# Sudaraka88/LDWeaver

Hardware: AMD Instinct MI355X
Metric: MI SNP-pairs/sec (higher is better)
Workload: dtype i8

## Files before the change

### ldweaver_amd/csrc/ldw_apx.hip

```cpp
#include <algorithm>
#include <cmath>
#include <cstdlib>
#include <cstring>

#include "ldw_apx.h"
#include "ldw_dev.h"

using namespace ldw;

namespace ldw {

namespace {
constexpr int64_t APX_PROD_CAP = 12000;
struct ProdTable {
    std::vector<int32_t> val;
    std::vector<uint8_t> a, b;
    ProdTable() {
        std::vector<std::pair<int32_t, std::pair<uint8_t, uint8_t>>> all;
        for (int x = 0; x <= 127; ++x)
            for (int y = x; y <= 127; ++y) all.push_back({x * y, {(uint8_t)x, (uint8_t)y}});
        std::sort(all.begin(), all.end());
        for (auto &e : all)
            if (val.empty() || val.back() != e.first) {
                val.push_back(e.first);
// ... 177 lines not shown
    const u64x2v q = {*reinterpret_cast<const uint64_t *>(lut_bytes + (d & 0xFFFFu)), *reinterpret_cast<const uint64_t *>(lut_bytes + (d >> 16))};
    return __builtin_bit_cast(v4i, q);
}
constexpr int APX_LUT_BYTES = 2048;

template <int MT, int NT>
__device__ __forceinline__ void apx_gemm_epilogue(const ApxGemmArgs &P, v16i (&acc)[MT][NT], int ty, int tx, int lane, const int2 *s_tab, uint8_t *s_bt) {
    constexpr int TH = 32 * MT, TWd = 32 * NT;
    const int frow = lane & 31, fh = lane >> 5;
    int bf[NT];
    if (P.fuse) {
#pragma unroll
        for (int j = 0; j < NT; ++j) bf[j] = (int)P.bin_f[tx * TWd + 32 * j + frow];
        for (int r = lane; r < TH; r += 64) s_bt[r] = P.bin_t[ty * TH + r];
        __builtin_amdgcn_wave_barrier();
        __builtin_amdgcn_s_waitcnt(0);
    }
#pragma unroll
    for (int i = 0; i < MT; ++i) {
        bool store = true;
        if (P.fuse) {
            bool ok = true;
#pragma unroll
            for (int j = 0; j < NT; ++j) ok = ok && bf[j] != 255;
            if (P.sr_mask && P.sr_mask[(int64_t)((ty * TH) / 128) * (P.RFpad / 64) + tx] != 0) ok = false;
            int bt[16];
#pragma unroll
            for (int e = 0; e < 16; ++e) {
                bt[e] = (int)s_bt[32 * i + (e & 3) + 8 * (e >> 2) + 4 * fh];
                ok = ok && bt[e] != 255;
            }
            unsigned int fails = 0;
            const bool eligible = __ballot(!ok) == 0ull;
            if (eligible) {
#pragma unroll
                for (int e = 0; e < 16; ++e)
#pragma unroll
                    for (int j = 0; j < NT; ++j) {
                        const int2 th = s_tab[bt[e] * P.tab_nb + bf[j]];
                        const int n = acc[i][j][e];
                        const bool in = n > th.x && n < th.y;
                        ok = ok && in;
                        if (!in) fails |= 1u << (e * NT + j);
                    }
            }
            if (NT == 2 && P.maybe && eligible && __ballot(!ok) != 0ull) {
                const unsigned int mine = (unsigned int)__popc(fails);
                unsigned int incl = mine;
#pragma unroll
                for (int o = 1; o < 64; o <<= 1) {
                    const unsigned int t = __shfl_up(incl, o);
                    if (lane >= o) incl += t;
                }
                const unsigned int tot = (unsigned int)__builtin_amdgcn_readlane((int)incl, 63);
                if (tot <= (unsigned int)APX_MAYBE_MAX) {
                    unsigned int base = 0;
                    if (lane == 0) base = atomicAdd(P.maybe_n, tot);
                    base = (unsigned int)__builtin_amdgcn_readfirstlane((int)base);
                    unsigned int pos = base + incl - mine;
                    unsigned int f = fails;
                    while (f) {
                        const int b = __builtin_ctz(f);
                        f &= f - 1;
                        const int e = b / NT, j = b % NT;
                        if (pos < P.maybe_cap) {
                            ApxMaybe m;
                            m.trow = (uint32_t)(ty * TH + 32 * i + (e & 3) + 8 * (e >> 2) + 4 * fh);
                            m.fcol = (uint32_t)(tx * TWd + 32 * j + frow);
                            int v = 0;
#pragma unroll
                            for (int ee = 0; ee < 16; ++ee)
#pragma unroll
                                for (int jj = 0; jj < NT; ++jj) v = (ee == e && jj == j) ? acc[i][jj][ee] : v;
                            m.n = v;
                            P.maybe[pos] = m;
                        }
                        ++pos;
                    }
                    ok = true;
                }
            }
#ifdef LDW_ABLATE_GEMM_STORE
            const bool clean = __ballot(bf[0] == 255 || bt[0] == 255) == 0ull || __ballot(!ok) == 0ull;
#else
            const bool clean = __ballot(!ok) == 0ull;
#endif
            if (lane == 0) {
#pragma unroll
                for (int h = 0; h < (NT * 32) / 64; ++h) P.clean[(int64_t)((ty * TH + 32 * i) / 32) * (P.RFpad / 64) + (tx * TWd) / 64 + h] = clean ? 1 : 0;
            }
            store = !clean;
        }
        if (store) {
#pragma unroll
            for (int j = 0; j < NT; ++j) {
                const int fcol = tx * TWd + 32 * j + frow;
#pragma unroll
                for (int e = 0; e < 16; ++e) {
                    const int trow = ty * TH + 32 * i + (e & 3) + 8 * (e >> 2) + 4 * fh;
                    P.G[(int64_t)trow * P.RFpad + fcol] = acc[i][j][e];
                }
            }
        }
    }
}

struct TileSummary {
    int bmin, bmax;
    unsigned fand, forr;
};
__device__ __forceinline__ TileSummary apx_fold_rows(const uint8_t *__restrict__ bins, const uint8_t *__restrict__ flags, int n) {
    TileSummary S{255, 0, 0xFFu, 0u};
    for (int i = 0; i < n; i += 16) {
        const uint4 b = *reinterpret_cast<const uint4 *>(bins + i);
        const unsigned w[4] = {b.x, b.y, b.z, b.w};
#pragma unroll
        for (int k = 0; k < 16; ++k) {
            const int v = (int)((w[k >> 2] >> (8 * (k & 3))) & 0xFFu);
            S.bmin = v < S.bmin ? v : S.bmin;
            S.bmax = v > S.bmax ? v : S.bmax;
        }
        if (flags) {
            const uint4 f = *reinterpret_cast<const uint4 *>(flags + i);
            unsigned a = f.x & f.y & f.z & f.w, o = f.x | f.y | f.z | f.w;
            a &= a >> 16; a &= a >> 8;
            o |= o >> 16; o |= o >> 8;
            S.fand &= a & 0xFFu;
            S.forr |= o & 0xFFu;
        }
    }
    return S;
}

__global__ __launch_bounds__(256) void k_apx_live_tiles(ApxGemmArgs P) {
    constexpr int MT = APX_MT, NT = 2, TH = 32 * MT, TWd = 32 * NT;
    __shared__ unsigned int s_wave[4], s_base;
    const int ty = (int)blockIdx.x, ntx = P.RFpad / TWd;
    const int lane = threadIdx.x & 63, wave = threadIdx.x >> 6;
    const TileSummary T = apx_fold_rows(P.bin_t + (int64_t)ty * TH, P.rflag_t ? P.rflag_t + (int64_t)ty * TH : nullptr, TH);
    unsigned int n_pruned = 0;
    for (int tx0 = 0; tx0 < ntx; tx0 += 256) {
        const int tx = tx0 + (int)threadIdx.x;
        const bool valid = tx < ntx && !(P.lower_only && tx * TWd + TWd - 1 < ty * TH);
        bool pruned = false, all_binned = false;
        if (valid && !(P.sr_mask && P.sr_mask[(int64_t)((ty * TH) / 128) * (P.RFpad / 64) + tx] != 0)) {
            const TileSummary F = apx_fold_rows(P.bin_f + (int64_t)tx * TWd, P.rflag_f ? P.rflag_f + (int64_t)tx * TWd : nullptr, TWd);
            all_binned = T.bmax < P.tab_nb && F.bmax < P.tab_nb;
            if (P.rflag_t) {
                const unsigned kt = T.fand & PF_KIND, kf = F.fand & PF_KIND;
                pruned = kt >= 2u && kt == (T.forr & PF_KIND) && kf >= 2u && kf == (F.forr & PF_KIND) &&
                         ((T.fand & (kf == 2u ? PF_DEAD2 : PF_DEAD3)) != 0u || (F.fand & (kt == 2u ? PF_DEAD2 : PF_DEAD3)) != 0u);
            }
            if (!pruned && all_binned && (T.bmax - T.bmin + 1) * (F.bmax - F.bmin + 1) <= 64) {
                bool ok = true;
                for (int bt = T.bmin; bt <= T.bmax; ++bt)
                    for (int bf = F.bmin; bf <= F.bmax; ++bf) {
                        const int2 th = P.tab[bt * P.tab_nb + bf];
                        ok = ok && th.x < 0 && th.y == 2147483647;
                    }
                pruned = ok;
            }
        }
        if (pruned && all_binned) {
#pragma unroll
            for (int i = 0; i < MT; ++i)
#pragma unroll
                for (int h = 0; h < (NT * 32) / 64; ++h) P.clean[(int64_t)((ty * TH + 32 * i) / 32) * (P.RFpad / 64) + (tx * TWd) / 64 + h] = 1;
        }
        const bool live = valid && !pruned;
        const unsigned long long lm = __ballot(live);
        n_pruned += (unsigned int)__popcll(__ballot(valid && pruned));
        if (lane == 0) s_wave[wave] = (unsigned int)__popcll(lm);
        __syncthreads();
        if (threadIdx.x == 0) {
            const unsigned int tot = s_wave[0] + s_wave[1] + s_wave[2] + s_wave[3];
            s_base = tot ? atomicAdd(P.n_live, tot) : 0u;
        }
        __syncthreads();
        unsigned int off = s_base;
        for (int w = 0; w < wave; ++w) off += s_wave[w];
        if (live) P.tile_list[off + (unsigned int)__popcll(lm & ((1ull << lane) - 1ull))] = (uint32_t)(ty * ntx + tx);
        __syncthreads();
    }
    if (lane == 0 && n_pruned) atomicAdd(P.skip_ctr, (unsigned long long)n_pruned);
}

template <int MT, int NT, bool FINE, int WPS = 2>
__global__ __launch_bounds__(256, WPS) void gemm_apx_kernel(ApxGemmArgs P) {
    extern __shared__ __attribute__((aligned(16))) uint8_t smem[];
    uint64_t *lutFF = reinterpret_cast<uint64_t *>(smem);
    uint8_t *sA = smem + APX_LUT_BYTES, *sB = sA + (size_t)P.M2 * 128;
    int2 *s_tab = reinterpret_cast<int2 *>(sB + (size_t)P.M2 * 128);
    const int tid = threadIdx.x;
    const int lane = tid & 63, wave = __builtin_amdgcn_readfirstlane(tid >> 6);
    constexpr int TH = 32 * MT, TWd = 32 * NT;
    const int ntx = P.RFpad / TWd;
    unsigned int k = 0, k_end = 0, step = 1;
    int t;
    if (P.tile_list) {
        const unsigned int n_live = *P.n_live, nw = gridDim.x * 4u, w = blockIdx.x * 4u + (unsigned int)wave;
        if (blockIdx.x * 4u >= n_live) return;
#ifdef LDW_APX_RUNS_CONTIG
        const unsigned int base = n_live / nw, rem = n_live % nw;
        k = w * base + (w < rem ? w : rem);
        k_end = k + base + (w < rem ? 1u : 0u);
#else
        k = w;
        k_end = n_live;
        step = nw;
#endif
        t = k < k_end ? (int)P.tile_list[k] : -1;
    } else {
        auto outside = [&](int ty, int tx) { return ty * TH >= P.RTpad || tx * TWd >= P.RFpad || (P.lower_only && tx * TWd + TWd - 1 < ty * TH); };
        const int ty0 = 2 * (int)blockIdx.y, tx0 = 2 * (int)blockIdx.x;
        if (outside(ty0, tx0) && outside(ty0, tx0 + 1) && outside(ty0 + 1, tx0) && outside(ty0 + 1, tx0 + 1)) return;
        const int ty = ty0 + (wave >> 1), tx = tx0 + (wave & 1);
        t = outside(ty, tx) ? -1 : ty * ntx + tx;
    }
    if (P.fuse)
        for (int i = tid; i < P.tab_nb * P.tab_nb; i += 256) s_tab[i] = P.tab[i];
    {
        uint64_t e = 0;
#pragma unroll
        for (int k8 = 0; k8 < 8; ++k8) e |= ((tid >> k8) & 1) ? (0xFFull << (8 * k8)) : 0ull;
        lutFF[tid] = e;
        const int n16 = P.M2 * 8;
        for (int i = tid; i < n16; i += 256) {
            reinterpret_cast<uint4 *>(sA)[i] = reinterpret_cast<const uint4 *>(P.dig_a)[i];
            reinterpret_cast<uint4 *>(sB)[i] = reinterpret_cast<const uint4 *>(P.dig_b)[i];
        }
    }
    __syncthreads();
    if (t < 0) return;
    const int frow = lane & 31, fh = lane >> 5;
    const int64_t sta = (int64_t)P.RTpad * 2, stb = (int64_t)P.RFpad * 2;
    const uint8_t *base_t, *base_f;
    const unsigned int lane_off = (unsigned int)(frow * 2 + fh) * 16u;
    auto piece = [&](const uint8_t *base, int64_t macro_step_bytes, int i) {
        return *reinterpret_cast<const apx_u32x4 *>(base + macro_step_bytes + 1024 * i);
    };
    apx_u32x4 wa[MT], wb[NT], na[MT], nb[NT];
    auto open_tile = [&](int ty, int tx) {
        base_t = reinterpret_cast<const uint8_t *>(P.panel_t) + (int64_t)ty * TH * 32 + lane_off;
        base_f = reinterpret_cast<const uint8_t *>(P.panel_f) + (int64_t)tx * TWd * 32 + lane_off;
#pragma unroll
        for (int i = 0; i < MT; ++i) na[i] = piece(base_t, 0, i);
#pragma unroll
        for (int i = 0; i < NT; ++i) nb[i] = piece(base_f, 0, i);
    };
    const uint8_t *lut_bytes = smem;
    int ty = t / ntx, tx = t - ty * ntx;
    open_tile(ty, tx);
    for (;;) {
        k += step;
        const int t_next = k < k_end ? (int)P.tile_list[k] : -1;
        v16i acc[MT][NT];
#pragma unroll
        for (int i = 0; i < MT; ++i)
#pragma unroll
            for (int j = 0; j < NT; ++j)
#pragma unroll
                for (int e = 0; e < 16; ++e) acc[i][j][e] = 0;
        for (int m = 0; m < P.M2; ++m) {
#pragma unroll
            for (int i = 0; i < MT; ++i) wa[i] = na[i];
#pragma unroll
            for (int i = 0; i < NT; ++i) wb[i] = nb[i];
            if (m + 1 < P.M2) {
#pragma unroll
                for (int i = 0; i < MT; ++i) na[i] = piece(base_t, (int64_t)(m + 1) * sta * 16, i);
#pragma unroll
                for (int i = 0; i < NT; ++i) nb[i] = piece(base_f, (int64_t)(m + 1) * stb * 16, i);
            }
            typedef const __attribute__((address_space(4))) v4i *shift_ptr;
            const v4i sh4 = ((shift_ptr)(uintptr_t)P.shift)[m];
            const int shk[4] = {sh4[0], sh4[1], sh4[2], sh4[3]};
            const uint8_t *dA = sA + m * 128 + fh * (FINE ? 16 : 64), *dB = sB + m * 128 + fh * (FINE ? 16 : 64);
            auto kstep = [&](auto KKc) {
                constexpr int kk = decltype(KKc)::value;
                const int sh = shk[kk];
                if ((FINE || kk == 0) && sh) {
#pragma unroll
                    for (int i = 0; i < MT; ++i)
#pragma unroll
                        for (int j = 0; j < NT; ++j)
#pragma unroll
                            for (int e = 0; e < 16; ++e) acc[i][j][e] = (int)((unsigned)acc[i][j][e] >> sh);
                }
                const v4i da = *reinterpret_cast<const v4i *>(dA + (FINE ? 32 : 16) * kk);
                const v4i db = *reinterpret_cast<const v4i *>(dB + (FINE ? 32 : 16) * kk);
                v4i fa[MT], fb[NT];
#pragma unroll
                for (int i = 0; i < MT; ++i) fa[i] = expand16s<kk>(lut_bytes, wa[i]) & da;
#pragma unroll
                for (int i = 0; i < NT; ++i) fb[i] = expand16s<kk>(lut_bytes, wb[i]) & db;
#pragma unroll
                for (int i = 0; i < MT; ++i)
#pragma unroll
                    for (int j = 0; j < NT; ++j) acc[i][j] = __builtin_amdgcn_mfma_i32_32x32x32_i8(fa[i], fb[j], acc[i][j], 0, 0, 0);
            };
            kstep(std::integral_constant<int, 0>{});
            kstep(std::integral_constant<int, 1>{});
            kstep(std::integral_constant<int, 2>{});
            kstep(std::integral_constant<int, 3>{});
        }
        const int ty_next = t_next / ntx, tx_next = t_next - ty_next * ntx;
        if (t_next >= 0) open_tile(ty_next, tx_next);
        int bt_off = wave * 256;
// ... 738 lines not shown
```

### ldweaver_amd/csrc/ldw_mi.hip

```cpp
#include <algorithm>
#include <chrono>
#include <cmath>
#include <cstring>
#include "ldw_prim.h"

#include "ldw_internal.h"
#include "ldw_dev.h"
#ifndef LDW_SCREEN_V
#define LDW_SCREEN_V 2
#endif
#ifndef LDW_SCREEN_WAVES
#define LDW_SCREEN_WAVES 6
#endif
#include "ldw_epi.h"
#include "ldw_pass_plan.h"
#include <future>

#include "ldw_apx.h"

using namespace ldw;

namespace ldw {
#include "ldw_mi_screen.inc"
#include "ldw_mi_eval.inc"
#include "ldw_mi_select.inc"
}

namespace {
#include "ldw_mi_block.inc"
#include "ldw_mi_items.inc"
#include "ldw_mi_pass.inc"
}

namespace ldw {
int ensure_streams(ldw_ctx *c) {
    if (c->streams_ready) return LDW_OK;
    const unsigned quiet = hipEventDisableTiming;
    LDW_HIP(c->copy_stream.ensure(hipStreamNonBlocking));
    for (int k = 0; k < LDW_NSLOT; ++k) {
        LDW_HIP(c->ev_up[k].ensure(quiet));
        LDW_HIP(c->ev_done[k].ensure(quiet));
        LDW_HIP(c->ev_pick[k].ensure(quiet));
        LDW_HIP(c->ev_gemm[k].ensure(quiet));
        if (int rc = c->pin_pick[k].reserve((size_t)LDW_SPAN_MAX * PICK_STRIDE + 64, "ensure_streams")) return rc;
    }
    LDW_HIP(c->ev_lrc.ensure(quiet));
    for (auto &e : c->ev_probe) LDW_HIP(e.ensure(quiet));
    if (int rc = c->pin_lrc.reserve(64, "ensure_streams")) return rc;
    {
        int lo_p = 0, hi_p = 0;
        LDW_HIP(hipDeviceGetStreamPriorityRange(&lo_p, &hi_p));
        LDW_HIP(c->gemm_stream.ensure(hipStreamNonBlocking, lo_p));
    }
    LDW_HIP(c->lr_st.ensure(hipStreamNonBlocking));
    for (auto &e : c->lr_ev) LDW_HIP(e.ensure(quiet));
    if (int rc = c->lr_counts.reserve(sizeof(int64_t) * 64, "ensure_streams")) return rc;
    if (int rc = c->lr_pin.reserve((size_t)32 << 20, "ensure_streams")) return rc;
    c->streams_ready = true;
    return LDW_OK;
}

int join_prepare(ldw_ctx *c) {
    if (!c) return LDW_OK;
    int rc = LDW_OK;
    for (int which = 0; which < 2; ++which) {
        std::thread &t = which == 0 ? c->prep_thread : c->prep_thread2;
        if (t.joinable()) t.join();
        int &trc = which == 0 ? c->prep_rc : c->prep_rc2;
        if (trc != LDW_OK && rc == LDW_OK) {
            rc = trc;
            set_error("side thread of %s: %s", which == 0 ? "ldw_ctx_create" : "ldw_ctx_reserve", (which == 0 ? c->prep_err : c->prep_err2).c_str());
        }
        trc = LDW_OK;
    }
    return rc;
}

int reserve_slot_buffers(ldw_ctx *c, int64_t Npad, int64_t blk, int64_t nseg) {
    const int64_t KW = Npad / 64;
    const SlotGeom g = slot_geom_estimate(blk, nseg);
    const size_t RF = (size_t)g.RFpad, RT = (size_t)g.RTpad;
    const size_t cap = pair_cap_for(g.nf, g.nt, g.nseg);
    const size_t one = (size_t)blk * (size_t)blk;
    for (int s = 0; s < LDW_NSLOT; ++s) {
        if (int rc = c->panel[s][0].reserve(RF * (size_t)KW * 16)) return rc;
        if (int rc = c->panel[s][1].reserve(RT * (size_t)KW * 16)) return rc;
        if (int rc = c->Gapx[s].reserve(RF * RT * 4)) return rc;
        if (int rc = UnitsLayout(g).reserve(c->apx_units[s])) return rc;
        if (int rc = PacksLayout(g).reserve(c->apx_packs[s])) return rc;
        if (int rc = MiniLayout(g).reserve(c->apx_mini[s])) return rc;
        if (int rc = PairsLayout((uint32_t)cap, maybe_cap_for(g.RTpad, g.RFpad)).reserve(c->pairs[s])) return rc;
        if (int rc = BinsLayout(g).reserve(c->apx_bins[s])) return rc;
        if (int rc = c->apx_clean[s].reserve((RT / 32) * (RF / 64) + 64)) return rc;
        if (int rc = c->hist[s].reserve((size_t)nseg * NBINS * 8)) return rc;
        const size_t cand = std::max<size_t>(one, (size_t)nseg * std::min<size_t>(one, (size_t)PAIR_PATHS * PAIR_SHARDS * cap));
        if (int rc = c->cand_key[s].reserve(cand * 8)) return rc;
        if (int rc = c->cand_val[s].reserve(cand * 8)) return rc;
        if (int rc = gx(c, s).reserve(RF * RF * 8)) return rc;
    }
    if (int rc = c->pair_sums.reserve((size_t)PAIR_PATHS * PAIR_SHARDS * cap * 16 * 8)) return rc;
    return LDW_OK;
}

void warm_mi() {
    hipFuncAttributes a;
    (void)hipFuncGetAttributes(&a, reinterpret_cast<const void *>(&k_zero4));
    (void)hipFuncGetAttributes(&a, reinterpret_cast<const void *>(&k_mi_screen<1, true>));
    (void)hipGetLastError();
}
}

extern "C" {

int ldw_mi_block(ldw_ctx *c, const int32_t *from_idx, int64_t nf, const int32_t *to_idx, int64_t nt, int quirk_mode,
                 double *MI_out, int on_device) {
    if (int rc = check_gpu(c)) return rc;
    LDW_REQUIRE(from_idx && to_idx && MI_out, LDW_ERR_ARG, "ldw_mi_block: null argument");
    LDW_REQUIRE(quirk_mode == LDW_QUIRK_REFERENCE || quirk_mode == LDW_QUIRK_INTENDED, LDW_ERR_ARG, "bad quirk mode");
    EmitArgs E;
    memset(&E, 0, sizeof(E));
    if (int rc = run_block_mi(c, from_idx, nf, to_idx, nt, quirk_mode, E)) return rc;
    LDW_HIP(hipMemcpyAsync(MI_out, c->MIblk.p, (size_t)nf * nt * 8, on_device ? hipMemcpyDeviceToDevice : hipMemcpyDeviceToHost,
                           c->stream));
    LDW_HIP(hipStreamSynchronize(c->stream));
    float t01 = 0, t12 = 0;
    LDW_HIP(hipEventElapsedTime(&t01, c->ev[0], c->ev[1]));
    LDW_HIP(hipEventElapsedTime(&t12, c->ev[1], c->ev[2]));
    c->last_ms[0] = t01;
    c->last_ms[1] = t12;
    c->last_ms[2] = 0;
    c->last_ms[3] = t01 + t12;
    return LDW_OK;
}

int ldw_joint_tables(ldw_ctx *c, const int32_t *pair_a, const int32_t *pair_b, int64_t np, int64_t *counts_out,
                     int64_t *fixed_out, int *frac_bits_out) {
    if (int rc = check_gpu(c)) return rc;
    LDW_REQUIRE(pair_a && pair_b && np > 0, LDW_ERR_ARG, "ldw_joint_tables: bad argument");
    if (int rc = join_prepare(c)) return rc;
    if (int rc = ensure_rows(c)) return rc;
    if (frac_bits_out) *frac_bits_out = c->wts.frac_bits;
    const int64_t CH = 1024;
    std::vector<int8_t> ones((size_t)c->Npad, 1);
    ldw::DevBuf d_ones, d_out, d_cmarg;
    int rc = LDW_OK;
    if ((rc = d_ones.reserve((size_t)c->Npad)) || (rc = d_out.reserve((size_t)CH * 25 * 8)) || (rc = d_cmarg.reserve((size_t)c->L * 40))) return rc;
    hipError_t he = hipMemcpyAsync(d_ones.p, ones.data(), ones.size(), hipMemcpyHostToDevice, c->stream);
    if (he != hipSuccess) return ldw::hip_fail(he, "memcpy ones", __FILE__, __LINE__);
    hipLaunchKernelGGL(k_slot_counts, dim3((unsigned)((c->L + 255) / 256)), dim3(256), 0, c->stream,
                       c->rows.counts.as<int32_t>(), c->rows.slot_meta.as<uint32_t>(), c->L, d_cmarg.as<int64_t>());
    for (int64_t p0 = 0; p0 < np && rc == LDW_OK; p0 += CH) {
        const int64_t n = std::min(CH, np - p0);
        SideLists SF, ST;
        if ((rc = build_side(c, pair_a + p0, n, SF))) break;
        if ((rc = build_side(c, pair_b + p0, n, ST))) break;
        const int RFpad = SF.Rpad, RTpad = ST.Rpad;
        if ((rc = upload_i32(c, c->rowlist_f, SF.rowlist)) || (rc = upload_i32(c, c->rowlist_t, ST.rowlist)) ||
            (rc = upload_i32(c, c->lrow_f, SF.lrow)) || (rc = upload_i32(c, c->lrow_t, ST.lrow)))
            break;
        std::vector<int32_t> vf(pair_a + p0, pair_a + p0 + n), vt(pair_b + p0, pair_b + p0 + n);
        if ((rc = upload_i32(c, c->idx_f, vf)) || (rc = upload_i32(c, c->idx_t, vt))) break;
        if (hipStreamSynchronize(c->stream) != hipSuccess) { rc = LDW_ERR_HIP; break; }
        if ((rc = c->G.reserve((size_t)RFpad * RTpad * 8))) break;
        for (int pass = 0; pass < 2 && rc == LDW_OK; ++pass) {
            int64_t *host_out = pass == 0 ? counts_out : fixed_out;
            if (!host_out) continue;
            rc = launch_gemm_bits(c, c->rows.Mbits.as<uint64_t>(), c->KW, c->rowlist_t.as<int32_t>(), RTpad, c->rowlist_f.as<int32_t>(), RFpad, c->G.as<int64_t>(),
                                  pass == 0 ? 1 : c->wts.nlimbs, pass == 0 ? d_ones.as<int8_t>() : c->wts.digits.as<int8_t>(), 0);
// ... 416 lines not shown
```

### ldweaver_amd/csrc/ldw_mi_items.inc

```

struct StageImage {
    struct Part {
        size_t off, bytes;
        const void *src;
        void (*point)(DevPtrs &, const char *);
    };
    Part part[18] = {};
    int n = 0;
    size_t bytes = 0;
    template <class T> static T elem_of(const T *DevPtrs::*);
    template <auto F> using Elem = decltype(elem_of(F));
    template <auto F> size_t array(const Elem<F> *src, size_t count) {
        part[n] = Part{bytes, count * sizeof(Elem<F>), src, [](DevPtrs &D, const char *p) { D.*F = reinterpret_cast<const Elem<F> *>(p); }};
        bytes = (bytes + part[n].bytes + 63) / 64 * 64;
        return part[n++].off;
    }
    void copy_to(char *image) const {
        for (int k = 0; k < n; ++k)
            if (part[k].src && part[k].bytes) memcpy(image + part[k].off, part[k].src, part[k].bytes);
    }
    void bind(DevPtrs &D, const char *image) const {
        for (int k = 0; k < n; ++k) part[k].point(D, image + part[k].off);
    }
};

struct HostBlock {
    int64_t nf = 0, nt = 0, n_sr_blk = 0, n_lr_total = 0, blk_no = 0;
    int RFpad = 0, RTpad = 0, slot = 0;
    bool diag = false, submitted = false;
    bool uploaded = false;
    bool mixed = false;
    bool apx = false;
    bool generic = false;
    int guess = -1;
    LoHost lo;
    StageImage img;
    size_t total = 0;
    DevPtrs D{};
    EmitArgs E{};
    int spec_B = -1;
    int span = 0;
    int32_t seg_start[LDW_SPAN_MAX] = {}, seg_nt[LDW_SPAN_MAX] = {};
    int64_t seg_lr_total[LDW_SPAN_MAX] = {};
    size_t cand_cap = 0;
    SpanSeg sseg[LDW_SPAN_MAX] = {};
    int pin_slot = -1;
    bool force_plain = false;
    bool span_alone = false;
    size_t stage_base = 0;
    int64_t sr_base = 0;
    std::vector<int32_t> span_from, span_to;
};

struct SpanPlan {
    int nseg = 0;
    int32_t start[LDW_SPAN_MAX] = {}, nt[LDW_SPAN_MAX] = {};
};

static inline bool speculation_pays(const ldw_ctx *c, const ldw_mi_params *p) {
    if (c->knobs.path_mode != 0) return true;
    return !(p->lr_links_approx > 0.0) || p->lr_retain_links < 0.007 * p->lr_links_approx;
}

struct PrepWork {
    ldw_ctx *c;
    const int32_t *from_idx, *to_idx;
    int64_t nf, nt;
    HostBlock &hb;
    std::vector<ColInfo> cols;
    std::string cols_err;
    std::future<int> cols_job;
    const std::vector<int32_t> *ord_f = nullptr, *ord_t = nullptr;
    std::vector<int32_t> ord_f_own, ord_t_own, ord_f_full, ord_t_full;
    SideLists SF, ST;
    std::vector<int32_t> pf, cmax, tf;
    std::vector<int64_t> tbase;
    std::vector<uint8_t> band;
    std::vector<uint32_t> bandl;
    int intervals(const ldw_mi_params *p, const SpanPlan *sp);
    int row_order(const SpanPlan *sp);
    void tiles(int slot);
    void band_mask();
    bool band_list();
    int join_cols() {
        const int rc = cols_job.valid() ? cols_job.get() : LDW_OK;
        if (rc != LDW_OK) set_error("%s", cols_err.c_str());
        return rc;
    }
    ~PrepWork() { if (cols_job.valid()) cols_job.wait(); }
};

int PrepWork::intervals(const ldw_mi_params *p, const SpanPlan *sp) {
    const int64_t blk_no = hb.blk_no;
    auto ascending = [&](const int32_t *idx, int64_t n) {
        for (int64_t k = 1; k < n; ++k)
            if (c->meta.h_POS[idx[k]] < c->meta.h_POS[idx[k - 1]]) return false;
        return true;
    };
    hb.generic = !ascending(from_idx, nf) || !ascending(to_idx, nt);
    if (hb.generic) {
        ColInfo z;
        memset(&z, 0, sizeof(z));
        cols.assign((size_t)nt, z);
        hb.n_sr_blk = 0;
    } else if (sp) {
        cols.resize((size_t)nt);
        std::vector<ColInfo> ck;
        for (int k = 0; k < sp->nseg; ++k) {
            int64_t n_k = 0;
            if (int rc = build_cols(c, from_idx, nf, to_idx + sp->start[k], sp->nt[k], false, p->sr_dist, ck, n_k)) return rc;
            std::copy(ck.begin(), ck.end(), cols.begin() + sp->start[k]);
        }
        hb.n_sr_blk = 0;
    } else if (hb.diag) {
        cols.resize((size_t)nt);
        const double sr_dist = p->sr_dist;
        cols_job = std::async(std::launch::async, [this, sr_dist]() -> int {
            const int rc = build_cols(c, from_idx, nf, to_idx, nt, true, sr_dist, cols, hb.n_sr_blk);
            if (rc != LDW_OK) cols_err = ldw_last_error();
            return rc;
        });
    } else if (int rc = build_cols(c, from_idx, nf, to_idx, nt, hb.diag, p->sr_dist, cols, hb.n_sr_blk)) return rc;
    if (sp) {
        LDW_REQUIRE(!hb.generic && !hb.diag && sp->nseg >= 1 && sp->nseg <= LDW_SPAN_MAX, LDW_ERR_STATE,
                    "span of %d blocks at block %lld cannot be formed", sp->nseg, (long long)blk_no);
        hb.span = sp->nseg;
        for (int k = 0; k < sp->nseg; ++k) {
            hb.seg_start[k] = sp->start[k];
            hb.seg_nt[k] = sp->nt[k];
            hb.seg_lr_total[k] = nf * (int64_t)sp->nt[k] - std::min<int64_t>(nf, sp->nt[k]);
            for (int32_t b = sp->start[k]; b < sp->start[k] + sp->nt[k]; ++b) {
                cols[(size_t)b].pad[0] = k;
                cols[(size_t)b].pad[1] = sp->start[k];
            }
        }
    }
    return LDW_OK;
}

int PrepWork::row_order(const SpanPlan *sp) {
    if (c->knobs.prune && !hb.generic && !hb.diag && c->knobs.engine == LDW_ENGINE_MFMA && c->apx.apx_ok) {
        bool rowless = false;
        for (int64_t k = 0; k < nf && !rowless; ++k) rowless = c->rows.h_row0[from_idx[k] + 1] == c->rows.h_row0[from_idx[k]];
        for (int64_t k = 0; k < nt && !rowless; ++k) rowless = c->rows.h_row0[to_idx[k] + 1] == c->rows.h_row0[to_idx[k]];
        if (!rowless) {
            ord_f = minor_weight_order(c, from_idx, nf, ord_f_full);
            ord_t = minor_weight_order(c, to_idx, nt, ord_t_full);
            if (hb.n_sr_blk > 0) {
                std::vector<int32_t> df((size_t)nf + 1, 0);
                std::vector<uint8_t> in_f((size_t)nf, 0), in_t((size_t)nt, 0);
                for (int64_t b = 0; b < nt; ++b)
                    for (int iv = 0; iv < 3; ++iv) {
                        const ColInfo &ci = cols[(size_t)b];
                        if (ci.e[iv] <= ci.s[iv]) continue;
                        in_t[(size_t)b] = 1;
                        ++df[(size_t)ci.s[iv]];
                        --df[(size_t)ci.e[iv]];
                    }
                int32_t run = 0;
                for (int64_t a = 0; a < nf; ++a) {
                    run += df[(size_t)a];
                    in_f[(size_t)a] = run > 0 ? 1 : 0;
                }
                auto rest_then_corner = [&](const std::vector<int32_t> &sorted, const std::vector<uint8_t> &corner, const int32_t *idx, int64_t n,
                                            std::vector<int32_t> &out) {
                    out.clear();
                    out.reserve(sorted.size());
                    for (int32_t k : sorted)
                        if (!corner[(size_t)k]) out.push_back(k);
                    for (int64_t k = 0; k < n; ++k)
                        if (corner[(size_t)k] && c->rows.h_row0[idx[k] + 1] - c->rows.h_row0[idx[k]] == 1) out.push_back((int32_t)k);
                };
                rest_then_corner(*ord_f, in_f, from_idx, nf, ord_f_own);
                rest_then_corner(*ord_t, in_t, to_idx, nt, ord_t_own);
                ord_f = &ord_f_own;
                ord_t = &ord_t_own;
            }
            c->cnt.sorted_blocks += sp ? sp->nseg : 1;
        }
    }
    LDW_REQUIRE(!sp || (ord_f && ord_t), LDW_ERR_STATE, "span at block %lld cannot be ordered", (long long)hb.blk_no);
    return LDW_OK;
}

void PrepWork::tiles(int slot) {
    build_perm_tiles(c, from_idx, nf, pf, ord_f);
    hb.D.nf_tiles = (int)(pf.size() / 64);
    {
        int64_t n12f = 0, n1 = 0, n2 = 0;
        for (int64_t k = 0; k < nf; ++k) {
            const int nr = c->rows.h_row0[from_idx[k] + 1] - c->rows.h_row0[from_idx[k]];
            n1 += nr == 1;
            n2 += nr == 2;
        }
        n12f = (n1 + 63) / 64 + (n2 + 63) / 64;
        hb.D.gen_t0 = (int)n12f;
        int64_t q12 = 0;
        for (int64_t k = 0; k < nt; ++k) {
            const int nr = c->rows.h_row0[to_idx[k] + 1] - c->rows.h_row0[to_idx[k]];
            q12 += nr == 1 || nr == 2;
        }
        hb.D.gen_q0 = (int)q12;
    }
    cmax.assign((size_t)hb.D.nf_tiles, 1);
    tbase.assign(cmax.size(), 0);
    {
        LoHost &lo = hb.lo;
        lo = LoHost();
        for (int64_t k = 0; k < nt; ++k) ++lo.n_lc[lo_class(c->rows.h_row0[to_idx[k] + 1] - c->rows.h_row0[to_idx[k]])];
        int32_t uo = 0, rb = 0;
        for (int lc = 0; lc < 3; ++lc) {
            lo.uoff[lc] = uo;
            lo.rowbase[lc] = rb;
            uo += lo.n_lc[lc];
            rb += (int32_t)((((int64_t)lo.n_lc[lc] << lc) + TILE - 1) / TILE * TILE);
        }
        lo.RTlo = rb;
        lo.ntiles = (int32_t)cmax.size();
        for (size_t t = 0; t < pf.size(); ++t) {
            if (pf[t] < 0) continue;
            const int32_t a = from_idx[pf[t]];
            const int cls = 1 << lo_class(c->rows.h_row0[a + 1] - c->rows.h_row0[a]);
            if (cls > cmax[t / 64]) cmax[t / 64] = cls;
        }
        int64_t tb = 0;
        for (size_t t = 0; t < cmax.size(); ++t) {
            tbase[t] = tb;
            tb += (int64_t)lo.RTlo * 64 * cmax[t];
            ++lo.n_tiles_cf[cmax[t] == 1 ? 0 : (cmax[t] == 2 ? 1 : 2)];
        }
        lo.slot = slot;
        lo.diag = hb.diag ? 1 : 0;
        lo.glo_total = tb;
    }
    for (size_t t = cmax.size(); t-- > 0;)
        for (int fs = 0; fs < cmax[t]; ++fs) {
            tf.push_back((int32_t)t);
            tf.push_back(fs);
        }
    hb.lo.n_tf = (int32_t)(tf.size() / 2);
}

void PrepWork::band_mask() {
    band.assign((size_t)(hb.RTpad / TILE) * (hb.RFpad / 64), 0);
    bool no_rowless = true;
    {
        const int ntx = hb.RFpad / 64;
        auto cls_of = [&](int32_t snp) { const int nr = c->rows.h_row0[snp + 1] - c->rows.h_row0[snp]; return nr <= 1 ? 0 : (nr == 2 ? 1 : 2); };
        std::vector<int32_t> pre[3];
        int32_t base[3] = {0, 0, 0};
        for (int k = 0; k < 3; ++k) pre[k].assign((size_t)nf + 1, 0);
        for (int64_t a = 0; a < nf; ++a) {
            const int k = cls_of(from_idx[a]);
            for (int q = 0; q < 3; ++q) pre[q][(size_t)a + 1] = pre[q][(size_t)a] + (q == k ? 1 : 0);
            const uint32_t m = c->rows.h_slot_meta[(size_t)from_idx[a]];
            const int n = (int)(m & 7);
            if ((n == 1 || n == 2) && (((m >> 3) & ((2u << n) - 1u)) != ((2u << n) - 1u))) hb.lo.band_full = 1;
            if (n == 0) hb.lo.band_full = 1;
            if (n == 0) no_rowless = false;
        }
        for (int64_t b2 = 0; b2 < nt; ++b2) {
            const uint32_t m = c->rows.h_slot_meta[(size_t)to_idx[b2]];
            const int n = (int)(m & 7);
            if (n == 0) no_rowless = false;
            if ((n == 1 || n == 2) && (((m >> 3) & ((2u << n) - 1u)) != ((2u << n) - 1u))) hb.lo.band_full = 1;
        }
        {
            int64_t rows = 0;
            for (int k = 0; k < 3; ++k) {
                base[k] = (int32_t)rows;
                rows += (int64_t)pre[k][(size_t)nf] * (1 << k);
                rows = (rows + 31) / 32 * 32;
            }
        }
        auto mark = [&](int64_t t0, int64_t t1, int64_t f0, int64_t f1) {
            for (int64_t ty = t0 / TILE; ty <= (t1 - 1) / TILE; ++ty)
                for (int64_t tx = f0 / 64; tx <= (f1 - 1) / 64; ++tx) band[(size_t)ty * ntx + tx] = 1;
        };
        std::vector<int32_t> nxt1, prv1;
        if (hb.n_sr_blk > 0 && !hb.lo.band_full && ord_f) {
            nxt1.assign((size_t)nf + 1, (int32_t)nf);
            prv1.assign((size_t)nf + 1, -1);
            for (int64_t a = nf - 1; a >= 0; --a) nxt1[(size_t)a] = cls_of(from_idx[a]) == 0 ? (int32_t)a : nxt1[(size_t)a + 1];
            for (int64_t a = 0; a < nf; ++a) prv1[(size_t)a + 1] = cls_of(from_idx[a]) == 0 ? (int32_t)a : prv1[(size_t)a];
        }
        if (hb.n_sr_blk > 0 && !hb.lo.band_full)
            for (int64_t b2 = 0; b2 < nt; ++b2) {
                const ColInfo &ci = cols[(size_t)b2];
                const int64_t rb0 = ST.lrow[(size_t)b2], rb1 = rb0 + (1 << cls_of(to_idx[b2]));
                for (int iv = 0; iv < 3; ++iv) {
                    if (ci.e[iv] <= ci.s[iv]) continue;
                    for (int k = 0; k < 3; ++k) {
                        const int32_t n0 = pre[k][(size_t)ci.s[iv]], n1 = pre[k][(size_t)ci.e[iv]];
                        if (n1 <= n0) continue;
                        int64_t f0 = base[k] + (int64_t)(n0 / 64 * 64) * (1 << k), f1 = base[k] + (int64_t)((n1 + 63) / 64 * 64) * (1 << k);
                        if (k == 0 && ord_f) {
                            const int64_t first = nxt1[(size_t)ci.s[iv]], last = prv1[(size_t)ci.e[iv]];
                            f0 = (int64_t)SF.lrow[(size_t)first] / 64 * 64;
                            f1 = ((int64_t)SF.lrow[(size_t)last] + 1 + 63) / 64 * 64;
                        }
                        if (k == 2) {
                            f0 = base[2];
                            f1 = base[2] + (int64_t)pre[2][(size_t)nf] * 4;
                        }
                        if (f1 > hb.RFpad) f1 = hb.RFpad;
                        mark(rb0, rb1, f0, f1);
                        if (hb.diag) mark(f0, f1, rb0, rb1);
                    }
                }
            }
    }
    hb.lo.fuse_ok = no_rowless ? 1 : 0;
    hb.lo.ordered = ord_f != nullptr ? 1 : 0;
}

bool PrepWork::band_list() {
    bool listed = false;
    const int64_t ntx = hb.RFpad / 64;
    if (hb.n_sr_blk > 0 && !hb.lo.band_full && hb.RTpad / TILE < 65536 && ntx < 65536) {
        const int64_t nty = hb.RTpad / TILE;
        for (int64_t ty = 0; ty < nty; ++ty)
            for (int64_t tx = 0; tx < ntx; ++tx)
                if (band[(size_t)ty * ntx + tx] && !(hb.diag && tx * 64 + 63 < ty * TILE)) bandl.push_back((uint32_t)(ty << 16 | tx));
        listed = bandl.size() * 2 <= band.size();
        if (!listed) bandl.clear();
    }
    hb.D.n_band = (int)bandl.size();
    return listed;
}

int prep_block(ldw_ctx *c, const int32_t *from_idx, int64_t nf, const int32_t *to_idx, int64_t nt, const ldw_mi_params *p,
               int slot, int64_t blk_no, HostBlock &hb, const SpanPlan *sp = nullptr, int pin_slot = -1, size_t stage_base = 0) {
    LDW_REQUIRE(nf > 0 && nt > 0, LDW_ERR_ARG, "empty block (nf=%lld nt=%lld)", (long long)nf, (long long)nt);
    LDW_REQUIRE(nf <= 1000000 && nt <= 1000000 && nf * nt < 2147483647LL, LDW_ERR_ARG, "block too large (%lld x %lld)",
                (long long)nf, (long long)nt);
    for (int64_t k = 0; k < nf; ++k)
        LDW_REQUIRE(from_idx[k] >= 0 && from_idx[k] < c->L, LDW_ERR_ARG, "SNP index %d out of range", from_idx[k]);
    for (int64_t k = 0; k < nt; ++k)
        LDW_REQUIRE(to_idx[k] >= 0 && to_idx[k] < c->L, LDW_ERR_ARG, "SNP index %d out of range", to_idx[k]);
    const bool prep_timing = ldw::host_timing();
    auto pnow = [] { return std::chrono::duration<double, std::micro>(std::chrono::steady_clock::now().time_since_epoch()).count(); };
    double tp[8] = {pnow(), 0, 0, 0, 0, 0, 0, 0};
    hb = HostBlock();
    hb.nf = nf;
    hb.nt = nt;
    hb.slot = slot;
    hb.blk_no = blk_no;
    hb.pin_slot = pin_slot;
    hb.stage_base = stage_base;
    hb.diag = same_list(from_idx, nf, to_idx, nt);
    PrepWork W{c, from_idx, to_idx, nf, nt, hb};
    if (int rc = W.intervals(p, sp)) return rc;
    tp[1] = pnow();
    if (int rc = W.row_order(sp)) return rc;
    tp[2] = pnow();
    if (int rc = build_side(c, from_idx, nf, W.SF, W.ord_f)) return rc;
    if (int rc = build_side(c, to_idx, nt, W.ST, W.ord_t)) return rc;
    tp[3] = pnow();
    hb.RFpad = W.SF.Rpad;
    hb.RTpad = W.ST.Rpad;
    W.tiles(slot);
    if (int rc = W.join_cols()) return rc;
    hb.n_lr_total = (hb.diag ? nf * (nf - 1) / 2 : nf * nt - std::min(nf, nt)) - hb.n_sr_blk;
    tp[4] = pnow();
    W.band_mask();
    tp[5] = pnow();
    const bool band_listed = W.band_list();
    StageImage &im = hb.img;
    im.array<&DevPtrs::idx_f>(from_idx, (size_t)nf);
    im.array<&DevPtrs::idx_t>(to_idx, (size_t)nt);
    im.array<&DevPtrs::rl_f>(W.SF.rowlist.data(), W.SF.rowlist.size());
    im.array<&DevPtrs::rl_t>(W.ST.rowlist.data(), W.ST.rowlist.size());
    im.array<&DevPtrs::lrow_f>(W.SF.lrow.data(), (size_t)nf);
    im.array<&DevPtrs::lrow_t>(W.ST.lrow.data(), (size_t)nt);
    im.array<&DevPtrs::perm>(W.pf.data(), W.pf.size());
    const size_t at_perm_t = im.array<&DevPtrs::perm_t>(nullptr, (size_t)nt);
    im.array<&DevPtrs::cols>(W.cols.data(), W.cols.size());
    im.array<&DevPtrs::pos_f>(W.SF.pos.data(), W.SF.pos.size());
    im.array<&DevPtrs::pos_t>(W.ST.pos.data(), W.ST.pos.size());
    im.array<&DevPtrs::cls_f>(W.SF.cls.data(), W.SF.cls.size());
    im.array<&DevPtrs::cls_t>(W.ST.cls.data(), W.ST.cls.size());
    im.array<&DevPtrs::cmax_f>(W.cmax.data(), W.cmax.size());
    im.array<&DevPtrs::tile_base>(W.tbase.data(), W.tbase.size());
    im.array<&DevPtrs::tf_list>(W.tf.data(), W.tf.size());
    im.array<&DevPtrs::band_mask>(W.band.data(), W.band.size());
    if (band_listed) im.array<&DevPtrs::band_list>(W.bandl.data(), W.bandl.size());
    hb.total = im.bytes;
    const int ps = pin_slot >= 0 ? pin_slot : slot;
    if (c->pin[ps].cap < stage_base + hb.total)
        if (int rc = c->pin[ps].reserve_keep((stage_base + hb.total) * 2, stage_base)) return rc;
    tp[6] = pnow();
    char *b = c->pin[ps].as<char>() + stage_base;
    im.copy_to(b);
    build_perm(c, to_idx, nt, reinterpret_cast<int32_t *>(b + at_perm_t), W.ord_t);
    if (prep_timing && blk_no < 12)
        fprintf(stderr, "[ldw prep us] block %lld%s %lld x %lld span %d: checks + intervals %.0f  row order %.0f  sides %.0f  tiles + classes %.0f  band %.0f  band list %.0f  copy to staging %.0f  (%zu bytes)\n",
                (long long)blk_no, hb.diag ? " diag" : "", (long long)nf, (long long)nt, hb.span, tp[1] - tp[0], tp[2] - tp[1], tp[3] - tp[2], tp[4] - tp[3], tp[5] - tp[4], tp[6] - tp[5], pnow() - tp[6], hb.total);
    return LDW_OK;
}

int launch_gather(ldw_ctx *c, const HostBlock &hb, const EmitArgs &E, const SmallLayout &sl) {
    GatherArgs S;
    S.MI = c->MIblk.as<double>();
    S.cols = E.cols;
    S.nf = (int)hb.nf;
    S.nt = (int)hb.nt;
    S.lower_only = E.lower_only;
    hipLaunchKernelGGL(k_lr_gather, dim3((unsigned)((hb.nt + 15) / 16)), dim3(256), 0, c->stream, S, sl.pick[hb.slot], E.ckey, E.cval);
    LDW_HIP(hipGetLastError());
    return LDW_OK;
}

double lo_bound(const ldw_ctx *c) {
    const double den = c->wts.neff > 1.0 ? c->wts.neff : 1.0;
    return c->wts.lo_abs_sum * (2.0 * std::log(den + 12.5) + 3.0) / den;
}

int make_emit_args(ldw_ctx *c, HostBlock &hb, const ldw_mi_params *p, const SmallLayout &sl, int spec_B) {
    const int s = hb.slot;
    const bool do_lr = !p->sr_only;
    EmitArgs E;
    memset(&E, 0, sizeof(E));
    E.cols = hb.D.cols;
    E.nf = (int)hb.nf;
    E.lower_only = hb.diag ? 1 : 0;
    E.keep_sr = p->keep_sr ? 1 : 0;
    E.do_lr = do_lr ? 1 : 0;
    E.sr_base = c->early_sr ? hb.sr_base : c->links.n_sr;
    E.sr_a = c->links.sr_a.as<int32_t>();
    E.sr_b = c->links.sr_b.as<int32_t>();
    E.sr_mi = c->links.sr_mi.as<double>();
    hb.spec_B = spec_B;
    size_t cap = (size_t)hb.nf * hb.nt;
    if (hb.span) {
        size_t seg_max = 0;
        for (int k = 0; k < hb.span; ++k) seg_max = std::max(seg_max, (size_t)hb.nf * (size_t)hb.seg_nt[k]);
        hb.cand_cap = std::min<size_t>(seg_max, (size_t)PAIR_PATHS * PAIR_SHARDS * pair_cap_for(hb.nf, hb.nt, hb.span));
        cap = hb.cand_cap * (size_t)hb.span;
    }
    if (do_lr && !hb.force_plain) {
        if (int rc = c->cand_key[s].reserve(cap * 8)) return rc;
        if (int rc = c->cand_val[s].reserve(cap * 8)) return rc;
    }
    if (hb.span) {
        if (int rc = c->hist[s].reserve((size_t)hb.span * NBINS * 8)) return rc;
        for (int k = 0; k < hb.span; ++k) {
            ldw::PickOut *pk = reinterpret_cast<ldw::PickOut *>(reinterpret_cast<char *>(sl.pick[s]) + (size_t)k * PICK_STRIDE);
            hb.sseg[k].n_cand = &pk->n_cand;
            hb.sseg[k].ckey = c->cand_key[s].as<uint64_t>() + (size_t)k * hb.cand_cap;
            hb.sseg[k].cval = c->cand_val[s].as<uint64_t>() + (size_t)k * hb.cand_cap;
            hb.sseg[k].ghist = c->hist[s].as<unsigned long long>() + (size_t)k * NBINS;
        }
    }
    E.write_dense = (do_lr && hb.spec_B < 0) ? 1 : 0;
    E.spec_B = hb.spec_B;
    E.spec_lo = hb.spec_B > 0 ? bucket_lo(hb.spec_B) : -1e300;
    E.any_sr = hb.n_sr_blk > 0 ? 1 : 0;
    E.n_cand = &sl.pick[s]->n_cand;
    E.ckey = c->cand_key[s].as<uint64_t>();
    E.cval = c->cand_val[s].as<uint64_t>();
    if (hb.force_plain && do_lr) {
        if (int rc = c->miss_key.reserve((size_t)hb.nf * hb.nt * 8)) return rc;
        if (int rc = c->miss_val.reserve((size_t)hb.nf * hb.nt * 8)) return rc;
        E.ckey = c->miss_key.as<uint64_t>();
        E.cval = c->miss_val.as<uint64_t>();
    }
    E.scr_mode = (hb.spec_B > 0 || !do_lr) && !E.write_dense && (!do_lr || speculation_pays(c, p)) ? c->knobs.screen : 0;
    const int64_t tot = hb.mixed ? c->wts.total_fixed_hi : c->wts.total_fixed;
    int bits = 0;
    while (bits < 62 && (tot >> bits) != 0) ++bits;
    E.scr_shift = bits > 31 ? bits - 31 : 0;
    E.scr_scale = (float)std::ldexp(1.0, E.scr_shift - c->wts.frac_bits + (hb.mixed ? 8 * LO_LIMBS : 0));
    E.scr_eps = SCREEN_EPS + (hb.mixed ? (float)lo_bound(c) : 0.0f);
    if (hb.apx) {
        apx_screen_params(c, E);
    }
// ... 587 lines not shown
```

Baseline: 175.7 billion.

## Tighten band tile mask with corner partitions and dedupe marks; early-exit APX pruning

Measured after the change: 176.4 billion, median of 3. No clear change (+0.4%).

```diff
diff --git a/ldweaver_amd/csrc/ldw_apx.hip b/ldweaver_amd/csrc/ldw_apx.hip
--- a/ldweaver_amd/csrc/ldw_apx.hip
+++ b/ldweaver_amd/csrc/ldw_apx.hip
@@ -353,8 +353,9 @@
                          ((T.fand & (kf == 2u ? PF_DEAD2 : PF_DEAD3)) != 0u || (F.fand & (kt == 2u ? PF_DEAD2 : PF_DEAD3)) != 0u);
             }
             if (!pruned && all_binned && (T.bmax - T.bmin + 1) * (F.bmax - F.bmin + 1) <= 64) {
-                bool ok = true;
-                for (int bt = T.bmin; bt <= T.bmax; ++bt)
+                const int2 far = P.tab[T.bmax * P.tab_nb + F.bmax];
+                bool ok = far.x < 0 && far.y == 2147483647;
+                for (int bt = T.bmin; ok && bt <= T.bmax; ++bt)
                     for (int bf = F.bmin; bf <= F.bmax; ++bf) {
                         const int2 th = P.tab[bt * P.tab_nb + bf];
                         ok = ok && th.x < 0 && th.y == 2147483647;
diff --git a/ldweaver_amd/csrc/ldw_band_tiles.h b/ldweaver_amd/csrc/ldw_band_tiles.h
--- /dev/null
+++ b/ldweaver_amd/csrc/ldw_band_tiles.h
@@ -0,0 +1,100 @@
+#pragma once
+#include <cstddef>
+#include <cstdint>
+#include <vector>
+#include "ldw_slots.h"
+
+namespace ldw {
+
+struct BandIn {
+    int64_t nf = 0, nt = 0;
+    const uint8_t *cls_f = nullptr, *cls_t = nullptr;
+    const int32_t *lrow_f = nullptr, *lrow_t = nullptr;
+    const uint8_t *part_f = nullptr;
+    int n_parts = 1;
+    const ColInfo *cols = nullptr;
+    bool diag = false;
+    int RFpad = 0, RTpad = 0;
+};
+constexpr int BAND_TILE_T = 128;
+
+inline void band_tiles(const BandIn &in, std::vector<uint8_t> &band) {
+    const int ntx = in.RFpad / 64;
+    const int64_t nf = in.nf;
+    band.assign((size_t)(in.RTpad / BAND_TILE_T) * (size_t)ntx, 0);
+    const int P = in.part_f ? in.n_parts : 1, NC = P + 2;
+    std::vector<int32_t> pre((size_t)(nf + 1) * NC, 0), mem, mem0((size_t)P + 1, 0);
+    for (int64_t a = 0; a < nf; ++a) {
+        const int k = in.cls_f[a], q = k == 0 ? (in.part_f ? (int)in.part_f[a] : 0) : P + k - 1;
+        int32_t *row = &pre[(size_t)(a + 1) * NC];
+        for (int j = 0; j < NC; ++j) row[j] = row[j - NC];
+        ++row[q];
+    }
+    const int32_t *tot = &pre[(size_t)nf * NC];
+    for (int p = 0; p < P; ++p) mem0[(size_t)p + 1] = mem0[(size_t)p] + tot[p];
+    mem.assign((size_t)mem0[(size_t)P], 0);
+    {
+        std::vector<int32_t> w(mem0.begin(), mem0.end() - 1);
+        for (int64_t a = 0; a < nf; ++a)
+            if (in.cls_f[a] == 0) mem[(size_t)w[in.part_f ? in.part_f[a] : 0]++] = (int32_t)a;
+    }
+    int64_t base[3];
+    {
+        int64_t rows = 0, n0 = 0;
+        for (int p = 0; p < P; ++p) n0 += tot[p];
+        const int64_t cnt[3] = {n0, tot[P], tot[P + 1]};
+        for (int k = 0; k < 3; ++k) {
+            base[k] = rows;
+            rows += cnt[k] * (1 << k);
+            rows = (rows + 31) / 32 * 32;
+        }
+    }
+    struct Rect {
+        int64_t ty0 = -1, ty1 = -1, tx0 = -1, tx1 = -1;
+    };
+    std::vector<Rect> last((size_t)3 * NC * 2);
+    auto mark = [&](Rect &was, int64_t t0, int64_t t1, int64_t f0, int64_t f1) {
+        const Rect r{t0 / BAND_TILE_T, (t1 - 1) / BAND_TILE_T, f0 / 64, (f1 - 1) / 64};
+        if (r.ty0 == was.ty0 && r.ty1 == was.ty1 && r.tx0 == was.tx0 && r.tx1 == was.tx1) return;
+        was = r;
+        for (int64_t ty = r.ty0; ty <= r.ty1; ++ty) {
+            uint8_t *row = &band[(size_t)ty * ntx];
+            for (int64_t tx = r.tx0; tx <= r.tx1; ++tx) row[tx] = 1;
+        }
+    };
+    for (int64_t b = 0; b < in.nt; ++b) {
+        const ColInfo &ci = in.cols[b];
+        const int64_t rb0 = in.lrow_t[b], rb1 = rb0 + (1 << in.cls_t[b]);
+        for (int iv = 0; iv < 3; ++iv) {
+            if (ci.e[iv] <= ci.s[iv]) continue;
+            const int32_t *ps = &pre[(size_t)ci.s[iv] * NC], *pe = &pre[(size_t)ci.e[iv] * NC];
+            for (int q = 0; q < NC; ++q) {
+                const int32_t n0 = ps[q], n1 = pe[q];
+                if (n1 <= n0) continue;
+                int64_t f0, f1;
+                if (q < P) {
+                    f0 = (int64_t)in.lrow_f[mem[(size_t)mem0[q] + n0]] / 64 * 64;
+                    f1 = ((int64_t)in.lrow_f[mem[(size_t)mem0[q] + n1 - 1]] + 1 + 63) / 64 * 64;
+                } else if (q == P) {
+                    f0 = base[1] + (int64_t)(n0 / 64 * 64) * 2;
+                    f1 = base[1] + (int64_t)((n1 + 63) / 64 * 64) * 2;
+                } else {
+                    f0 = base[2];
+                    f1 = base[2] + (int64_t)tot[P + 1] * 4;
+                }
+                if (f1 > in.RFpad) f1 = in.RFpad;
+                mark(last[(size_t)(iv * NC + q) * 2], rb0, rb1, f0, f1);
+                if (in.diag) mark(last[(size_t)(iv * NC + q) * 2 + 1], f0, f1, rb0, rb1);
+            }
+        }
+    }
+}
+
+inline void band_tile_list(const std::vector<uint8_t> &band, int64_t nty, int64_t ntx, bool diag, std::vector<uint32_t> &list) {
+    list.clear();
+    for (int64_t ty = 0; ty < nty; ++ty)
+        for (int64_t tx = 0; tx < ntx; ++tx)
+            if (band[(size_t)ty * ntx + tx] && !(diag && tx * 64 + 63 < ty * BAND_TILE_T)) list.push_back((uint32_t)(ty << 16 | tx));
+}
+
+}
diff --git a/ldweaver_amd/csrc/ldw_mi.hip b/ldweaver_amd/csrc/ldw_mi.hip
--- a/ldweaver_amd/csrc/ldw_mi.hip
+++ b/ldweaver_amd/csrc/ldw_mi.hip
@@ -14,6 +14,7 @@
 #endif
 #include "ldw_epi.h"
 #include "ldw_pass_plan.h"
+#include "ldw_band_tiles.h"
 #include <future>
 
 #include "ldw_apx.h"
diff --git a/ldweaver_amd/csrc/ldw_mi_items.inc b/ldweaver_amd/csrc/ldw_mi_items.inc
--- a/ldweaver_amd/csrc/ldw_mi_items.inc
+++ b/ldweaver_amd/csrc/ldw_mi_items.inc
@@ -72,6 +72,9 @@
     std::future<int> cols_job;
     const std::vector<int32_t> *ord_f = nullptr, *ord_t = nullptr;
     std::vector<int32_t> ord_f_own, ord_t_own, ord_f_full, ord_t_full;
+    const uint8_t *part_f = nullptr;
+    int n_parts = 1;
+    std::vector<uint8_t> corner_f;
     SideLists SF, ST;
     std::vector<int32_t> pf, cmax, tf;
     std::vector<int64_t> tbase;
@@ -175,6 +178,9 @@
                 rest_then_corner(*ord_t, in_t, to_idx, nt, ord_t_own);
                 ord_f = &ord_f_own;
                 ord_t = &ord_t_own;
+                corner_f.swap(in_f);
+                part_f = corner_f.data();
+                n_parts = 2;
             }
             c->cnt.sorted_blocks += sp ? sp->nseg : 1;
         }
@@ -242,73 +248,39 @@
 }
 
 void PrepWork::band_mask() {
-    band.assign((size_t)(hb.RTpad / TILE) * (hb.RFpad / 64), 0);
     bool no_rowless = true;
-    {
-        const int ntx = hb.RFpad / 64;
-        auto cls_of = [&](int32_t snp) { const int nr = c->rows.h_row0[snp + 1] - c->rows.h_row0[snp]; return nr <= 1 ? 0 : (nr == 2 ? 1 : 2); };
-        std::vector<int32_t> pre[3];
-        int32_t base[3] = {0, 0, 0};
-        for (int k = 0; k < 3; ++k) pre[k].assign((size_t)nf + 1, 0);
-        for (int64_t a = 0; a < nf; ++a) {
-            const int k = cls_of(from_idx[a]);
-            for (int q = 0; q < 3; ++q) pre[q][(size_t)a + 1] = pre[q][(size_t)a] + (q == k ? 1 : 0);
-            const uint32_t m = c->rows.h_slot_meta[(size_t)from_idx[a]];
-            const int n = (int)(m & 7);
-            if ((n == 1 || n == 2) && (((m >> 3) & ((2u << n) - 1u)) != ((2u << n) - 1u))) hb.lo.band_full = 1;
-            if (n == 0) hb.lo.band_full = 1;
-            if (n == 0) no_rowless = false;
-        }
-        for (int64_t b2 = 0; b2 < nt; ++b2) {
-            const uint32_t m = c->rows.h_slot_meta[(size_t)to_idx[b2]];
-            const int n = (int)(m & 7);
-            if (n == 0) no_rowless = false;
-            if ((n == 1 || n == 2) && (((m >> 3) & ((2u << n) - 1u)) != ((2u << n) - 1u))) hb.lo.band_full = 1;
-        }
-        {
-            int64_t rows = 0;
-            for (int k = 0; k < 3; ++k) {
-                base[k] = (int32_t)rows;
-                rows += (int64_t)pre[k][(size_t)nf] * (1 << k);
-                rows = (rows + 31) / 32 * 32;
-            }
-        }
-        auto mark = [&](int64_t t0, int64_t t1, int64_t f0, int64_t f1) {
-            for (int64_t ty = t0 / TILE; ty <= (t1 - 1) / TILE; ++ty)
-                for (int64_t tx = f0 / 64; tx <= (f1 - 1) / 64; ++tx) band[(size_t)ty * ntx + tx] = 1;
-        };
-        std::vector<int32_t> nxt1, prv1;
-        if (hb.n_sr_blk > 0 && !hb.lo.band_full && ord_f) {
-            nxt1.assign((size_t)nf + 1, (int32_t)nf);
-            prv1.assign((size_t)nf + 1, -1);
-            for (int64_t a = nf - 1; a >= 0; --a) nxt1[(size_t)a] = cls_of(from_idx[a]) == 0 ? (int32_t)a : nxt1[(size_t)a + 1];
-            for (int64_t a = 0; a < nf; ++a) prv1[(size_t)a + 1] = cls_of(from_idx[a]) == 0 ? (int32_t)a : prv1[(size_t)a];
-        }
-        if (hb.n_sr_blk > 0 && !hb.lo.band_full)
-            for (int64_t b2 = 0; b2 < nt; ++b2) {
-                const ColInfo &ci = cols[(size_t)b2];
-                const int64_t rb0 = ST.lrow[(size_t)b2], rb1 = rb0 + (1 << cls_of(to_idx[b2]));
-                for (int iv = 0; iv < 3; ++iv) {
-                    if (ci.e[iv] <= ci.s[iv]) continue;
-                    for (int k = 0; k < 3; ++k) {
-                        const int32_t n0 = pre[k][(size_t)ci.s[iv]], n1 = pre[k][(size_t)ci.e[iv]];
-                        if (n1 <= n0) continue;
-                        int64_t f0 = base[k] + (int64_t)(n0 / 64 * 64) * (1 << k), f1 = base[k] + (int64_t)((n1 + 63) / 64 * 64) * (1 << k);
-                        if (k == 0 && ord_f) {
-                            const int64_t first = nxt1[(size_t)ci.s[iv]], last = prv1[(size_t)ci.e[iv]];
-                            f0 = (int64_t)SF.lrow[(size_t)first] / 64 * 64;
-                            f1 = ((int64_t)SF.lrow[(size_t)last] + 1 + 63) / 64 * 64;
-                        }
-                        if (k == 2) {
-                            f0 = base[2];
-                            f1 = base[2] + (int64_t)pre[2][(size_t)nf] * 4;
-                        }
-                        if (f1 > hb.RFpad) f1 = hb.RFpad;
-                        mark(rb0, rb1, f0, f1);
-                        if (hb.diag) mark(f0, f1, rb0, rb1);
-                    }
-                }
-            }
+    auto look = [&](const int32_t *idx, int64_t n, std::vector<uint8_t> &cls) {
+        cls.resize((size_t)n);
+        for (int64_t a = 0; a < n; ++a) {
+            const uint32_t m = c->rows.h_slot_meta[(size_t)idx[a]];
+            const int nr = (int)(m & 7);
+            cls[(size_t)a] = (uint8_t)(nr <= 1 ? 0 : (nr == 2 ? 1 : 2));
+            if ((nr == 1 || nr == 2) && (((m >> 3) & ((2u << nr) - 1u)) != ((2u << nr) - 1u))) hb.lo.band_full = 1;
+            if (nr == 0) hb.lo.band_full = 1;
+            if (nr == 0) no_rowless = false;
+        }
+    };
+    std::vector<uint8_t> cls_f, cls_t;
+    look(from_idx, nf, cls_f);
+    look(to_idx, nt, cls_t);
+    if (hb.n_sr_blk > 0 && !hb.lo.band_full) {
+        BandIn in;
+        in.nf = nf;
+        in.nt = nt;
+        in.cls_f = cls_f.data();
+        in.cls_t = cls_t.data();
+        in.lrow_f = SF.lrow.data();
+        in.lrow_t = ST.lrow.data();
+        in.part_f = ord_f ? part_f : nullptr;
+        in.n_parts = n_parts;
+        in.cols = cols.data();
+        in.diag = hb.diag;
+        in.RFpad = hb.RFpad;
+        in.RTpad = hb.RTpad;
+        static_assert(TILE == BAND_TILE_T, "band tiles are TILE to-side rows");
+        band_tiles(in, band);
+    } else {
+        band.assign((size_t)(hb.RTpad / TILE) * (hb.RFpad / 64), 0);
     }
     hb.lo.fuse_ok = no_rowless ? 1 : 0;
     hb.lo.ordered = ord_f != nullptr ? 1 : 0;
@@ -318,10 +290,7 @@
     bool listed = false;
     const int64_t ntx = hb.RFpad / 64;
     if (hb.n_sr_blk > 0 && !hb.lo.band_full && hb.RTpad / TILE < 65536 && ntx < 65536) {
-        const int64_t nty = hb.RTpad / TILE;
-        for (int64_t ty = 0; ty < nty; ++ty)
-            for (int64_t tx = 0; tx < ntx; ++tx)
-                if (band[(size_t)ty * ntx + tx] && !(hb.diag && tx * 64 + 63 < ty * TILE)) bandl.push_back((uint32_t)(ty << 16 | tx));
+        band_tile_list(band, hb.RTpad / TILE, ntx, hb.diag, bandl);
         listed = bandl.size() * 2 <= band.size();
         if (!listed) bandl.clear();
     }
```
